# TorontoDeepLearning/convnet

Measured on NVIDIA H100. Metric: images/sec ImageNet AlexNet training, higher is better.
Workload: dtype bf16

## Files before the change

convnet_b200/csrc/conv_tc.cu:

```cuda
#include <cuda.h>
#include <cuda_bf16.h>
#include <cudaTypedefs.h>

#include <algorithm>
#include <vector>

#include "conv_kernels.h"
#include "sm90_ptx.cuh"

namespace cnb {

namespace {

constexpr int kConsumerWarps = 8;
template <int SW> constexpr int kThreadsFor = 32 * (kConsumerWarps + 1 + SW);
constexpr int BM = 128;
constexpr int BN_MAX = 128;
constexpr int BK = 32;
constexpr int kMaxStages = 8;
constexpr uint32_t kAStageBytes = BM * 128;
constexpr uint32_t kBStageBytes = BN_MAX * 128;

enum Op { kFprop = 0, kDgrad = 1, kWgrad = 2 };

struct TcParams {
  int bf16, chunk, chunk_shift, cpt, bk, nbc;
  int N, nb;
  int W, H, modX, modY, modules;
  int Cin, Cout;
  int kx, ky, sx, sy, px, py, taps;
  int frames, frame0;
  int BN, stages;
  int m_tiles, n_tiles, num_tiles;
  int kc_blocks;
  int x_mode, x_yblocks, x_ct;
  const float* xw;
  uint32_t bank_bytes;
  uint32_t epi_bytes;
  uint32_t b_tx_bytes;
  int a_merged, b_merged;
  int untied;
  int total_chunks;
  int splits, units_per_split;
  long long part_stride;
// ... 181 lines not shown
  ptx::wgmma_fence_operands(acc);
}

__device__ __forceinline__ uint32_t epi_off(int row, int col) {
  return (uint32_t)(col * (BM * 4) + ((((row >> 2) ^ col) & 7) << 4) + (((row >> 2) & ~7) << 4) + ((row & 3) << 2));
}

constexpr int kWgradPassCols = 32;
constexpr uint32_t kWgradWarpBytes = 16 * kWgradPassCols * 4;
constexpr uint32_t kWgradStageBytes = kConsumerWarps * kWgradWarpBytes;
__device__ __forceinline__ uint32_t wgrad_stage_off(int row, int col) {
  return (uint32_t)(col * 64 + ((((row >> 2) ^ (col >> 1)) & 3) << 4) + ((row & 3) << 2));
}

__device__ __forceinline__ float4 ld4(const float* a, bool vec) {
  if (vec) return *reinterpret_cast<const float4*>(a);
  return make_float4(a[0], a[1], a[2], a[3]);
}
__device__ __forceinline__ float4 ldg4(const float* a, bool vec) {
  if (vec) return __ldg(reinterpret_cast<const float4*>(a));
  return make_float4(__ldg(a), __ldg(a + 1), __ldg(a + 2), __ldg(a + 3));
}

template <int OP, bool SIG, int SW>
__device__ __forceinline__ void store_tiles(const TcParams& p, SmemCtl* ctl, uint32_t stg, int sw, int lane) {
  constexpr int kStoreWarps = SW;
  constexpr int kEpiCols = (SW == 3 && !SIG) ? 8 : 4;
  const bool vec = p.vec != 0;
  const int lr = 4 * lane;
  const int per_frame = (OP == kFprop) ? p.modules : p.W * p.H;
  const long long col_stride = (long long)p.N * (OP == kFprop ? p.out_plane : (long long)per_frame);
  const bool direct_scale = p.splits == 1;
  const float so_eff = direct_scale ? p.so : 1.f;
  const bool rmw = direct_scale && p.st != 0.f;
  uint32_t phase = 0;
  for (int t = blockIdx.x; t < p.num_tiles; t += gridDim.x) {
    const Tile tile = decode_tile<OP>(p, t);
    long long row = -1;
    const int q = tile.m_tile * p.cpt + (lr >> p.chunk_shift);
    if (q < p.total_chunks) {
      const int ib = q % p.nbc, rr = q / p.nbc, pos = rr % per_frame, f = rr / per_frame;
      const int n = ib * p.chunk + (lr & (p.chunk - 1));
      if (n < p.N) {
        if (OP == kFprop) {
          const int i = pos % p.modX, j = pos / p.modX;
          const long long pix = (long long)(i * p.o_sx + p.o_x0) + (long long)p.o_W * (j * p.o_sy + p.o_y0);
          row = f * p.out_frame_step + n + (long long)p.N * pix;
        } else {
          row = n + (long long)p.N * pos;
        }
        row += col_stride * ((long long)tile.n_tile * p.BN) + tile.split * p.part_stride;
      }
    }
    const int ncols = min(p.BN, (OP == kFprop ? p.Cout : p.Cin) - tile.n_tile * p.BN);
    const float* bias = (OP == kFprop && p.bias) ? p.bias + tile.n_tile * p.BN : nullptr;
    int bias_step = 1;
    if (OP == kFprop && p.bias && p.untied) {
      bias = p.bias + (tile.m_tile * p.cpt / p.nbc) + (long long)p.modules * tile.n_tile * p.BN;
      bias_step = p.modules;
    }
    const int mine = ncols > sw ? (ncols - sw + kStoreWarps - 1) / kStoreWarps : 0;
    const int batches = (mine + kEpiCols - 1) / kEpiCols;
    static_assert(BN_MAX <= 64 * kStoreWarps, "two bias values per lane cover a store warp's columns");
    constexpr bool kBiasHi = BN_MAX > 32 * kStoreWarps;
    float bias_lo = 0.f, bias_hi = 0.f;
    if (OP == kFprop && bias) {
      const int ca = sw + kStoreWarps * lane, cb = ca + kStoreWarps * 32;
      if (ca < ncols) bias_lo = __ldg(bias + ca * bias_step);
      if (kBiasHi && cb < ncols) bias_hi = __ldg(bias + cb * bias_step);
    }
    float4 acc[kEpiCols], old[kEpiCols], msk[kEpiCols];
    auto load_batch = [&](int b) {
      const int c0 = sw + kStoreWarps * kEpiCols * b;
#pragma unroll
      for (int k = 0; k < kEpiCols; k++) {
        const int col = c0 + kStoreWarps * k;
        old[k] = msk[k] = make_float4(0.f, 0.f, 0.f, 0.f);
        if (row < 0 || col >= ncols) continue;
        const long long idx = row + col_stride * col;
        if (rmw) old[k] = ld4(p.out + idx, vec);
        if (p.mask) msk[k] = ldg4(p.mask + idx, vec);
      }
    };
    if (batches > 0) load_batch(0);
    ptx::mbar_wait(&ctl->epi_full, phase);
    if (batches == 0 && lane == 0) ptx::mbar_arrive(&ctl->epi_empty);
    for (int b = 0; b < batches; b++) {
// ... 53 lines not shown
          *reinterpret_cast<float4*>(dst) = acc[k];
        } else {
#pragma unroll
          for (int e = 0; e < 4; e++) dst[e] = v[e];
        }
        if (p.out16) {
          __nv_bfloat16* const d16 = p.out16 + idx;
          const __nv_bfloat162 lo = __floats2bfloat162_rn(v[0], v[1]), hi = __floats2bfloat162_rn(v[2], v[3]);
          if (vec) {
            uint2 w;
            w.x = *reinterpret_cast<const uint32_t*>(&lo);
            w.y = *reinterpret_cast<const uint32_t*>(&hi);
            *reinterpret_cast<uint2*>(d16) = w;
          } else {
            d16[0] = lo.x; d16[1] = lo.y; d16[2] = hi.x; d16[3] = hi.y;
          }
        }
      }
    }
    phase ^= 1;
  }
}

template <int OP, bool BF16, bool SIG, int SW>
__global__ void __launch_bounds__(kThreadsFor<SW>, 1)
tc_conv_kernel(const __grid_constant__ CUtensorMap mapA, const __grid_constant__ CUtensorMap mapB, const __grid_constant__ TcParams p) {
  extern __shared__ uint8_t smem_raw[];
  uint8_t* smem = reinterpret_cast<uint8_t*>((reinterpret_cast<uintptr_t>(smem_raw) + 1023) & ~uintptr_t(1023));
  uint8_t* smemA = smem;
  uint8_t* smemB = smem + (size_t)p.stages * kAStageBytes;
  uint8_t* smemE = smemB + (p.bank_bytes ? (size_t)p.bank_bytes : (size_t)p.stages * kBStageBytes);
  SmemCtl* ctl = reinterpret_cast<SmemCtl*>(smemE + p.epi_bytes);

  const int warp = __shfl_sync(0xffffffffu, (int)(threadIdx.x >> 5), 0), lane = threadIdx.x & 31;

  if (threadIdx.x == 0) {
    for (int s = 0; s < p.stages; s++) { ptx::mbar_init(&ctl->full[s], 1); ptx::mbar_init(&ctl->empty[s], kConsumerWarps); }
    ptx::mbar_init(&ctl->epi_full, kConsumerWarps);
    ptx::mbar_init(&ctl->epi_empty, SW);
    ptx::fence_barrier_init();
    ptx::tma_prefetch_desc(&mapA);
    ptx::tma_prefetch_desc(&mapB);
  }
  __syncthreads();
  ptx::pdl_launch_dependents();
  ptx::pdl_wait();

  if (warp > kConsumerWarps) {
    if constexpr (OP != kWgrad) store_tiles<OP, SIG, SW>(p, ctl, ptx::smem_u32(smemE), warp - kConsumerWarps - 1, lane);
    return;
  }
  if (warp == kConsumerWarps) {
    if (lane != 0) return;
    int stage = 0; uint32_t phase = 0;
    const uint32_t tx_bytes = kAStageBytes + p.b_tx_bytes;
    for (int t = blockIdx.x; t < p.num_tiles; t += gridDim.x) {
      const Tile tile = decode_tile<OP>(p, t);
      auto begin_stage = [&]() -> uint8_t* {
        ptx::mbar_wait(&ctl->empty[stage], phase ^ 1);
        ptx::mbar_arrive_expect_tx(&ctl->full[stage], tx_bytes);
        return smemA + (size_t)stage * kAStageBytes;
      };
      auto lda5 = [&](const void* m, void* dst, int c0, int c1, int c2, int c3, int c4) {
        ptx::tma_load_5d(m, &ctl->full[stage], dst, c0, c1, c2, c3, c4);
      };
      auto lda4 = [&](const void* m, void* dst, int c0, int c1, int c2, int c3) {
        ptx::tma_load_4d(m, &ctl->full[stage], dst, c0, c1, c2, c3);
      };
      auto lda3 = [&](const void* m, void* dst, int c0, int c1, int c2) {
        ptx::tma_load_3d(m, &ctl->full[stage], dst, c0, c1, c2);
      };
      auto end_stage = [&]() { if (++stage == p.stages) { stage = 0; phase ^= 1; } };
// ... 8 lines not shown
        }
        if (p.x_mode) {
          for (int c = 0; c < p.Cin; c++)
            for (int yb = 0; yb < p.x_yblocks; yb++) {
              uint8_t* a = begin_stage();
              if (p.a_merged) {
                lda5(&mapA, a, 0, cX[0], cY[0] + 4 * yb, ch.n[0] >> 5, c);
              } else {
#pragma unroll
                for (int q = 0; q < 4; q++)
                  lda5(&mapA, a + q * (BK * 128), ch.n[q], c, cX[q], cY[q] + 4 * yb, ch.f[q]);
              }
              end_stage();
            }
        } else {
          const int cb0 = p.splits > 1 ? tile.split * p.units_per_split : 0;
          const int cb1 = p.splits > 1 ? min(cb0 + p.units_per_split, p.kc_blocks) : p.kc_blocks;
          const int mod = ch.pos[0];
          for (int ty = 0; ty < p.ky; ty++)
            for (int tx = 0; tx < p.kx; tx++) {
              const int tap = tx + p.kx * ty;
              for (int cb = cb0; cb < cb1; cb++) {
                uint8_t* a = begin_stage();
                uint8_t* b = smemB + (size_t)stage * kBStageBytes;
                if (p.a_merged) {
                  lda5(&mapA, a, 0, cb * p.bk, ch.n[0] >> p.chunk_shift, cX[0] + tx, cY[0] + ty);
                } else {
#pragma unroll
                  for (int c = 0; c < 4; c++)
                    if (c < p.cpt) lda5(&mapA, a + c * (p.bk * 128), ch.n[c], cb * p.bk, cX[c] + tx, cY[c] + ty, ch.f[c]);
                }
                const int o0 = tile.n_tile * p.BN;
                if (p.b_merged) {
                  if (p.untied) lda5(&mapB, b, 0, cb * p.bk, o0 >> p.chunk_shift, tap, mod);
                  else lda4(&mapB, b, 0, cb * p.bk, o0 >> p.chunk_shift, tap);
                } else {
                  for (int j = 0; j < ((p.BN + p.chunk - 1) >> p.chunk_shift); j++) {
                    if (p.untied) lda4(&mapB, b + j * (p.bk * 128), o0 + j * p.chunk, tap, cb * p.bk, mod);
                    else lda3(&mapB, b + j * (p.bk * 128), o0 + j * p.chunk, tap, cb * p.bk);
                  }
                }
                end_stage();
              }
            }
        }
      } else if (OP == kDgrad) {
        const Chunks ch = decode_chunks(p, tile.m_tile, p.W * p.H);
        const DgradTaps taps = dgrad_taps(p, ch);
        const bool none = dgrad_live_taps(p, taps) == 0;
        int cX[4], cY[4];
#pragma unroll
        for (int c = 0; c < 4; c++) { cX[c] = ch.pos[c] % p.W; cY[c] = ch.pos[c] / p.W; }
        const int ob0 = p.splits > 1 ? tile.split * p.units_per_split : 0;
        const int ob1 = p.splits > 1 ? min(ob0 + p.units_per_split, p.kc_blocks) : p.kc_blocks;
        for (int ty = 0; ty < p.ky; ty++)
          for (int tx = 0; tx < p.kx; tx++) {
            if (!(taps.any(tx, ty) || (none && tx == 0 && ty == 0))) continue;
            int mx[4], my[4];
#pragma unroll
            for (int c = 0; c < 4; c++) {
              const bool lv = ch.ok[c] && taps.live(c, tx, ty);
              mx[c] = lv ? (cX[c] - p.px - tx) / p.sx : -1;
              my[c] = lv ? (cY[c] - p.py - ty) / p.sy : -1;
            }
            const int tap = tx + p.kx * ty;
            const int mod = mx[0] >= 0 ? mx[0] + p.modX * my[0] : -1;
            for (int ob = ob0; ob < ob1; ob++) {
              uint8_t* a = begin_stage();
              uint8_t* b = smemB + (size_t)stage * kBStageBytes;
              if (p.a_merged) {
                lda5(&mapA, a, 0, ob * p.bk, ch.n[0] >> p.chunk_shift, mx[0], my[0]);
              } else {
#pragma unroll
                for (int c = 0; c < 4; c++)
                  if (c < p.cpt) lda5(&mapA, a + c * (p.bk * 128), ch.n[c], ob * p.bk, mx[c], my[c], p.frame0);
              }
              if (p.untied) lda4(&mapB, b, ob * p.bk, tap, tile.n_tile * p.BN, mod);
              else lda3(&mapB, b, ob * p.bk, tap, tile.n_tile * p.BN);
              end_stage();
            }
          }
      } else if (p.untied) {
        const int mx = tile.split % p.modX, my = tile.split / p.modX;
        const int X = mx * p.sx + p.px + tile.tap % p.kx, Y = my * p.sy + p.py + tile.tap / p.kx;
        for (int ib = 0; ib < p.nbc; ib++) {
          uint8_t* a = begin_stage();
          uint8_t* b = smemB + (size_t)stage * kBStageBytes;
          lda5(&mapA, a, ib * p.chunk, mx, my, tile.o_tile * BM, 0);
          lda5(&mapB, b, ib * p.chunk, X, Y, tile.c_tile * p.BN, 0);
          end_stage();
        }
      } else if (p.x_mode) {
        const int r0 = tile.split * p.units_per_split, r1 = min(r0 + p.units_per_split, p.modY * p.frames);
        const uint32_t c_bytes = (uint32_t)p.ky * 8 * 128;
        for (int r = r0; r < r1; r++) {
          const int f = r / p.modY, my = r % p.modY;
          for (int mx = 0; mx < p.modX; mx++)
            for (int ib = 0; ib < p.nb; ib++) {
              uint8_t* a = begin_stage();
              uint8_t* b = smemB + (size_t)stage * kBStageBytes;
              lda5(&mapA, a, ib * 32, mx, my, tile.o_tile * BM, f);
              for (int c = 0; c < p.x_ct; c++)
                lda5(&mapB, b + c * c_bytes, ib * 32, mx * p.sx + p.px, my * p.sy + p.py, tile.c_tile * p.x_ct + c, f);
              end_stage();
            }
        }
      } else {
        const WgradSpan sp = wgrad_span(p, tile);
        const int tx = tile.tap % p.kx, ty = tile.tap / p.kx;
        if (sp.live_rows == 0 || sp.mx_hi < sp.mx_lo) {
          for (int ib = 0; ib < p.nbc; ib++) {
            uint8_t* a = begin_stage();
            uint8_t* b = smemB + (size_t)stage * kBStageBytes;
            lda5(&mapA, a, ib * p.chunk, 0, 0, tile.o_tile * BM, 0);
            lda5(&mapB, b, ib * p.chunk, -1, -1, tile.c_tile * p.BN, 0);
            end_stage();
          }
        } else {
          for (int r = sp.r0; r < sp.r1; r++) {
            if (!wgrad_row_live(p, r, ty)) continue;
            const int f = r / p.modY, my = r % p.modY;
            const int Y = my * p.sy + p.py + ty;
            for (int mx = sp.mx_lo; mx <= sp.mx_hi; mx++) {
              const int X = mx * p.sx + p.px + tx;
              for (int ib = 0; ib < p.nbc; ib++) {
                uint8_t* a = begin_stage();
                uint8_t* b = smemB + (size_t)stage * kBStageBytes;
                lda5(&mapA, a, ib * p.chunk, mx, my, tile.o_tile * BM, f);
                lda5(&mapB, b, ib * p.chunk, X, Y, tile.c_tile * p.BN, f);
                end_stage();
              }
            }
          }
        }
      }
    }
    return;
  }

  const int g = lane >> 2, tq = lane & 3;
  const int row0 = warp * 16 + g;
  int stage = 0; uint32_t phase = 0;
  int bank_tile = -1;
  uint32_t epi_phase = 0;
  for (int t = blockIdx.x; t < p.num_tiles; t += gridDim.x) {
    const Tile tile = decode_tile<OP>(p, t);
    const int nkb = tile_kblocks<OP>(p, tile);
    float acc[BN_MAX / 8][4];
#pragma unroll
    for (int j = 0; j < BN_MAX / 8; j++)
#pragma unroll
      for (int e = 0; e < 4; e++) acc[j][e] = 0.f;

    if constexpr (BF16 || OP == kWgrad) {
      constexpr bool a_mn = (OP != kWgrad), b_mn = (OP == kFprop);
      constexpr uint32_t a_step = a_mn ? 2048u : 32u, b_step = b_mn ? 2048u : 32u;
      const uint64_t da0 = ptx::gmma_desc(ptx::smem_u32(smemA) + (uint32_t)(warp >> 2) * 8192u, a_mn ? 8192u : 16u, 1024u);
      const uint64_t db0 = ptx::gmma_desc(ptx::smem_u32(smemB), b_mn ? 8192u : 16u, 1024u);
      int prev = -1;
      ptx::wgmma_fence_operands(acc);
      for (int kb = 0; kb < nkb; kb++) {
        ptx::mbar_wait(&ctl->full[stage], phase);
        ptx::wgmma_fence();
        const uint64_t da = da0 + ((uint32_t)stage * kAStageBytes >> 4), db = db0 + ((uint32_t)stage * kBStageBytes >> 4);
#pragma unroll
        for (int ks = 0; ks < 4; ks++) {
          if constexpr (BF16)
            ptx::wgmma_m64n128k16_bf16<a_mn ? 1 : 0, b_mn ? 1 : 0>(acc, da + (ks * a_step >> 4), db + (ks * b_step >> 4));
          else
            ptx::wgmma_m64n128k8_tf32(acc, da + (ks * a_step >> 4), db + (ks * b_step >> 4));
        }
        ptx::wgmma_commit();
        ptx::wgmma_wait<1>();
        if (prev >= 0 && lane == 0) ptx::mbar_arrive(&ctl->empty[prev]);
        prev = stage;
        if (++stage == p.stages) { stage = 0; phase ^= 1; }
      }
      ptx::wgmma_wait<0>();
      ptx::wgmma_fence_operands(acc);
      if (prev >= 0 && lane == 0) ptx::mbar_arrive(&ctl->empty[prev]);
    } else if (OP == kFprop && p.x_mode) {
      if (tile.n_tile != bank_tile) {
        ptx::bar_sync(1, 32 * kConsumerWarps);
        xmode_fill_bank(p, smemB, tile.n_tile);
        ptx::fence_proxy_async_smem();
        ptx::bar_sync(1, 32 * kConsumerWarps);
        bank_tile = tile.n_tile;
      }
      const uint32_t sA = ptx::smem_u32(smemA), bank = ptx::smem_u32(smemB);
      switch (p.BN) {
        case 32: xmode_fprop_mma<32>(acc, p, ctl, sA, bank, nkb, stage, phase, row0, tq, lane); break;
        case 64: xmode_fprop_mma<64>(acc, p, ctl, sA, bank, nkb, stage, phase, row0, tq, lane); break;
        case 96: xmode_fprop_mma<96>(acc, p, ctl, sA, bank, nkb, stage, phase, row0, tq, lane); break;
        default: xmode_fprop_mma<128>(acc, p, ctl, sA, bank, nkb, stage, phase, row0, tq, lane); break;
      }
    } else {
      const uint32_t sA = ptx::smem_u32(smemA), sB = ptx::smem_u32(smemB);
      constexpr bool b_mn = (OP == kFprop);
      for (int kb = 0; kb < nkb; kb++) {
        ptx::mbar_wait(&ctl->full[stage], phase);
        const uint32_t A = sA + (uint32_t)stage * kAStageBytes, B = sB + (uint32_t)stage * kBStageBytes;
#pragma unroll
        for (int ks = 0; ks < 4; ks++) {
          const int k0 = ks * 8 + tq, k1 = k0 + 4;
          const uint32_t a0 = ptx::lds32(A + off_mnmajor(row0, k0));
          const uint32_t a1 = ptx::lds32(A + off_mnmajor(row0 + 8, k0));
          const uint32_t a2 = ptx::lds32(A + off_mnmajor(row0, k1));
          const uint32_t a3 = ptx::lds32(A + off_mnmajor(row0 + 8, k1));
#pragma unroll
          for (int j = 0; j < BN_MAX / 8; j++) {
            if (j * 8 >= p.BN) break;
            const int n = j * 8 + g;
            const uint32_t b0 = ptx::lds32(B + (b_mn ? off_mnmajor(n, k0) : off_kmajor(n, k0)));
            const uint32_t b1 = ptx::lds32(B + (b_mn ? off_mnmajor(n, k1) : off_kmajor(n, k1)));
            ptx::mma_tf32_16x8x8(acc[j], a0, a1, a2, a3, b0, b1);
          }
        }
        __syncwarp();
        if (lane == 0) ptx::mbar_arrive(&ctl->empty[stage]);
        if (++stage == p.stages) { stage = 0; phase ^= 1; }
      }
    }

    if constexpr (OP != kWgrad) {
      ptx::mbar_wait(&ctl->epi_empty, epi_phase ^ 1);
      uint32_t base[2][2];
#pragma unroll
      for (int h = 0; h < 2; h++)
#pragma unroll
        for (int e = 0; e < 2; e++) base[h][e] = ptx::smem_u32(smemE) + epi_off(row0 + 8 * h, 2 * tq + e);
#pragma unroll
      for (int j = 0; j < BN_MAX / 8; j++) {
        if (j * 8 >= p.BN) break;
#pragma unroll
        for (int h = 0; h < 2; h++)
#pragma unroll
          for (int e = 0; e < 2; e++) ptx::sts32(base[h][e] + j * 8 * BM * 4, acc[j][2 * h + e]);
      }
      __syncwarp();
      if (lane == 0) ptx::mbar_arrive(&ctl->epi_full);
      epi_phase ^= 1;
    } else if (p.epi_bytes) {
      const uint32_t stg = ptx::smem_u32(smemE) + (uint32_t)warp * kWgradWarpBytes;
      const int r4 = 4 * (lane & 3);
      const int o = tile.o_tile * BM + warp * 16 + r4;
      const long long col_stride = (long long)p.Cout * p.taps;
      float* const rp = p.out + (long long)tile.split * p.Cout * p.taps * p.Cin + o + (long long)p.Cout * tile.tap +
                        col_stride * ((long long)tile.c_tile * p.BN);
      const int ncols_valid = min(p.BN, p.Cin - tile.c_tile * p.BN);
      const bool direct_scale = (p.splits == 1) || p.untied;
      const float so_eff = direct_scale ? p.so : 1.f;
      const bool rmw = direct_scale && p.st != 0.f;
#pragma unroll
      for (int pass = 0; pass < BN_MAX / kWgradPassCols; pass++) {
        if (pass * kWgradPassCols >= p.BN) break;
// ... 97 lines not shown
  if ((reinterpret_cast<uintptr_t>(base) & 15) != 0) return false;
  for (int i = 0; i < rank; i++) {
    if (dims[i] <= 0 || dims[i] > 0xFFFFFFFFLL) return false;
    gdim[i] = (cuuint64_t)dims[i];
    bdim[i] = (cuuint32_t)box[i];
    estr[i] = 1;
    if (box[i] > 256) return false;
    if (i > 0) {
      const long long bytes = strides[i - 1] * e.esz;
      if (bytes % 16 != 0 || bytes <= 0 || bytes >= (1LL << 40)) return false;
      gstr[i - 1] = (cuuint64_t)bytes;
    }
  }
  CUresult r = encode_fn()(map, e.bf16 ? CU_TENSOR_MAP_DATA_TYPE_BFLOAT16 : CU_TENSOR_MAP_DATA_TYPE_FLOAT32, (cuuint32_t)rank,
                           const_cast<void*>(base), gdim, gstr, bdim, estr, CU_TENSOR_MAP_INTERLEAVE_NONE,
                           CU_TENSOR_MAP_SWIZZLE_128B, CU_TENSOR_MAP_L2_PROMOTION_L2_256B, CU_TENSOR_MAP_FLOAT_OOB_FILL_NONE);
  if (r != CUDA_SUCCESS) {
    fprintf(stderr, "convnet_b200: cuTensorMapEncodeTiled failed (%d)\n", (int)r);
    return false;
  }
  return true;
}

int pick_bn(int cols, int granule) {
  const int tiles = ceil_div(cols, BN_MAX);
  const int bn = ceil_div(ceil_div(cols, tiles), granule) * granule;
  return std::min(BN_MAX, std::max(granule, bn));
}

size_t smem_bytes_for(int stages, uint32_t bank_bytes, uint32_t epi_bytes) {
  const size_t b = bank_bytes ? (size_t)bank_bytes : (size_t)stages * kBStageBytes;
  return 1024 + (size_t)stages * kAStageBytes + b + epi_bytes + sizeof(SmemCtl) + 16;
}
constexpr size_t kSmemBudget = 227 * 1024;
inline uint32_t epi_bytes_for(int bn) { return (uint32_t)BM * bn * 4; }

int pick_stages(uint32_t bank_bytes, uint32_t epi_bytes) {
  int s = kMaxStages;
  while (s > 2 && smem_bytes_for(s, bank_bytes, epi_bytes) > kSmemBudget) s--;
  return s;
}

int pick_store_warps(int kblocks, double tile_bytes) {
  const double mma_us = 0.3 * kblocks;
  const double epi_us = tile_bytes / (3e6 / 132);
  return 2.0 * epi_us >= mma_us ? 7 : 3;
}

template <int OP, bool BF16, bool SIG, int SW>
void launch_one(const CUtensorMap& a, const CUtensorMap& b, const TcParams& p, size_t smem) {
  smem_opt_in(tc_conv_kernel<OP, BF16, SIG, SW>, 227 * 1024);
  const int grid = std::min(p.num_tiles, num_sms());
  launch_pdl(tc_conv_kernel<OP, BF16, SIG, SW>, dim3((unsigned)grid), dim3(kThreadsFor<SW>), smem, state().stream, a, b, p);
}

template <int OP>
void launch(const CUtensorMap& a, const CUtensorMap& b, TcParams& p) {
  auto aligned = [](const void* q, uintptr_t a) { return (reinterpret_cast<uintptr_t>(q) & (a - 1)) == 0; };
  if (OP == kWgrad) p.epi_bytes = (!p.x_mode && p.Cout % 4 == 0 && aligned(p.out, 16)) ? kWgradStageBytes : 0u;
  else p.epi_bytes = epi_bytes_for(p.BN);
  p.stages = pick_stages(p.bank_bytes, p.epi_bytes);
  const size_t smem = smem_bytes_for(p.stages, p.bank_bytes, p.epi_bytes);
  p.vec = aligned(p.out, 16) && aligned(p.mask, 16) && aligned(p.out16, 8) ? 1 : 0;
  const bool sig = p.act == kActLogistic || (p.mask && p.mask_act == kActLogistic);
  CNB_REQUIRE(OP != kWgrad || !sig, "tc_conv: wgrad has no activation epilogue");
  void (*run)(const CUtensorMap&, const CUtensorMap&, const TcParams&, size_t) = nullptr;
  if constexpr (OP != kWgrad) {
    const int kcb = p.splits > 1 ? p.units_per_split : p.kc_blocks;
    const int kblocks = (OP == kFprop && p.x_mode) ? p.Cin * p.x_yblocks : p.taps * kcb;
    const double bytes = BM * p.BN * (4.0 + (p.out16 ? 2 : 0) + (p.mask ? 4 : 0) + (p.st != 0.f && p.splits == 1 ? 4 : 0));
    if (pick_store_warps(kblocks, bytes) == 7) {
      if (sig) run = p.bf16 ? launch_one<OP, true, true, 7> : launch_one<OP, false, true, 7>;
      else run = p.bf16 ? launch_one<OP, true, false, 7> : launch_one<OP, false, false, 7>;
    } else if (sig) {
      run = p.bf16 ? launch_one<OP, true, true, 3> : launch_one<OP, false, true, 3>;
    }
  }
  if (!run) run = p.bf16 ? launch_one<OP, true, false, 3> : launch_one<OP, false, false, 3>;
  run(a, b, p, smem);
  count_launch();
  CNB_LAUNCH_CHECK("tc_conv");
}

void fill_common(TcParams& p, const ConvGeom& g, const Elem& e) {
  p.bf16 = e.bf16; p.chunk = e.chunk; p.chunk_shift = e.shift; p.cpt = BM / e.chunk; p.bk = e.bk;
  p.N = g.N; p.nb = ceil_div(g.N, 32); p.nbc = ceil_div(g.N, e.chunk);
  p.W = g.W; p.H = g.H; p.modX = g.modX; p.modY = g.modY; p.modules = g.modules;
  p.Cin = g.Cin; p.Cout = g.Cout;
  p.kx = g.kx; p.ky = g.ky; p.sx = g.sx; p.sy = g.sy; p.px = g.px; p.py = g.py; p.taps = g.kx * g.ky;
  p.frames = g.frames; p.frame0 = 0;
  p.splits = 1; p.units_per_split = 0; p.part_stride = 0;
  p.x_mode = 0; p.x_yblocks = 0; p.x_ct = 0; p.b_tx_bytes = 0;
  p.xw = nullptr; p.bank_bytes = 0; p.epi_bytes = 0;
  p.a_merged = 0; p.b_merged = 0;
// ... 97 lines not shown
             st, so, bias, per_channel / 4, act, (const float4*)mask, mask_act);
  count_launch();
  CNB_LAUNCH_CHECK("reduce_split");
}
void set_tiles(TcParams& p, int total_chunks, int cols, int k_channels) {
  p.kc_blocks = ceil_div(k_channels, p.bk);
  p.total_chunks = total_chunks;
  p.m_tiles = ceil_div(p.total_chunks, p.cpt);
  p.n_tiles = ceil_div(cols, p.BN);
  p.num_tiles = p.m_tiles * p.n_tiles;
  p.b_tx_bytes = p.x_mode ? 0u : (uint32_t)p.BN * 128;
}
size_t split_k(TcParams& p, const ConvGeom& g, long long out_elems, bool allowed) {
  if (!allowed || p.x_mode || p.taps != 1 || g.frames != 1 || out_elems % 4 != 0) return 0;
  if (p.num_tiles * 2 > num_sms() || p.kc_blocks < 8) return 0;
  const int ks = std::max(std::min(num_sms() / p.num_tiles, p.kc_blocks / 4), 1);
  if (ks > 1) {
    p.units_per_split = ceil_div(p.kc_blocks, ks);
    p.splits = ceil_div(p.kc_blocks, p.units_per_split);
    p.part_stride = out_elems;
    p.num_tiles *= p.splits;
  }
  return p.splits > 1 ? align_up(sizeof(float) * out_elems * p.splits) : 0;
}

}

static ConvOutcome tc_conv_up_impl(const ConvGeom& g, const float* images, const float* filters, float* targets, float st,
                                   float so, const Fuse& fuse, __nv_bfloat16* out16, bool bf) {
  const Elem e = elem_for(bf);
  if (g.N % 4 != 0 || g.Cout % 4 != 0) return {};
  const bool x_mode = g.Cin < 8;
  if (x_mode && (g.kx > 8 || g.ky > 8)) return {};
  if (bf && (x_mode || g.N % 8 != 0 || g.Cout % 8 != 0 || !aligned16(images) || !aligned16(filters))) return {};
  if (!g.conv && (g.N % 128 != 0 || g.frames != 1 || x_mode)) return {};
  const long long flt_n = filter_elems(g);
  if (bf && (long long)g.N * g.modules * g.frames < 1024 && !bf16_staged(filters, flt_n)) return {};
  TcParams p; fill_common(p, g, e);
  p.BN = pick_bn(g.Cout, e.chunk);
  p.x_mode = x_mode ? 1 : 0;
  p.x_yblocks = ceil_div(g.ky, 4);
  if (x_mode) {
    auto bank_bytes = [&](int bn) { return (uint32_t)g.Cin * p.x_yblocks * bn * 128; };
    while (p.BN > 32 && smem_bytes_for(3, bank_bytes(p.BN), epi_bytes_for(p.BN)) > kSmemBudget) p.BN = ceil_div(p.BN / 2, 32) * 32;
    p.bank_bytes = bank_bytes(p.BN);
    p.xw = filters;
  }
  const long long chunks = (long long)p.nb * g.modules * g.frames;
  if (chunks * 4 >= (1LL << 31)) return {};
  set_tiles(p, p.nbc * g.modules * g.frames, g.Cout, g.Cin);
  float* const out = targets + (long long)g.cout0 * g.modules * g.N;
  const float* const bias = fuse.bias ? fuse.bias + (long long)g.cout0 * (g.conv ? 1 : g.modules) : nullptr;
  const long long out_elems = (long long)g.Cout * g.modules * g.N;
  const size_t part_bytes = split_k(p, g, out_elems, g.conv);
  p.out = out;
  p.st = st; p.so = so;
  p.bias = bias; p.act = fuse.act;
  CUtensorMap ma, mb;
  const CallBuffers buf = call_buffers(bf, part_bytes, {images, g.img_total, (long long)g.cin0 * g.H * g.W * g.N},
                                       {filters, flt_n, 0});
  const long long taps = (long long)g.kx * g.ky;
  if (p.splits > 1) { p.out = buf.part; p.bias = nullptr; p.act = 0; }
  const bool emit = out16 != nullptr && p.splits == 1 && g.cout0 == 0 && g.Cout == g.CoutT;
  if (emit) p.out16 = out16;
  const bool drop = fuse.drop_scale != 0.f && p.splits == 1 && g.frames == 1 && g.cout0 == 0 && g.Cout == g.CoutT;
  if (drop) { p.drop_prob = fuse.drop_prob; p.drop_scale = fuse.drop_scale; p.drop_seed = fuse.drop_seed; }
  p.a_merged = (g.frames == 1 && g.N % 128 == 0) ? 1 : 0;
  p.b_merged = (g.Cout % e.chunk == 0) ? 1 : 0;
  if (x_mode) {
    const long long N = g.N;
    if (p.a_merged) {
      if (!merged_image_map(&ma, buf.x, e, g, g.W, g.H, g.Cin, true)) return {};
    } else {
      const long long adims[5] = {N, g.Cin, g.W, g.H, g.frames};
      const long long astr[4] = {N * g.W * g.H, N, N * g.W, g.in_frame_step};
      const int abox[5] = {32, 1, 8, 4, 1};
      if (!make_map(&ma, buf.x, e, 5, adims, astr, abox)) return {};
    }
    mb = ma;
  } else {
    if (p.a_merged) {
      if (!merged_image_map(&ma, buf.x, e, g, g.W, g.H, g.Cin, false)) return {};
    } else if (!image_map(&ma, buf.x, e, g, g.W, g.H, g.Cin, g.in_frame_step, true, e.bk)) return {};
    if (!filter_map(&mb, buf.y, e, g.Cout, taps, g.Cin, p.BN, p.b_merged, g.conv ? 0 : g.modules)) return {};
  }
  launch<kFprop>(ma, mb, p);
  if (p.splits > 1)
    reduce_split(buf.part, out, out_elems, p.splits, st, so, bias, (long long)g.modules * g.N, fuse.act, nullptr, 0);
  return {bf ? kPathTcBf16 : kPathTcTf32, emit, drop};
// ... 28 lines not shown
                                         float so, const Fuse& fuse, __nv_bfloat16* out16) {
  DgradBanks banks;
  if (!dgrad_as_fprop_eligible(g, derivs, filters, &banks)) return {};
  const Elem e = elem_for(true);
  const __nv_bfloat16* sd = bf16_staged(derivs, g.out_total);
  if (!sd) {
    __nv_bfloat16* tmp = (__nv_bfloat16*)workspace(align_up((size_t)g.out_total * 2));
    to_bf16(derivs, tmp, g.out_total);
    sd = tmp;
  }
  const __nv_bfloat16* bank = dgrad_weights(filters, g, banks, false);
  for (int i = 0; i < banks.count; i++) {
    const DgradPhase& P = banks.phase[i];
    TcParams p; fill_common(p, g, e);
    p.modX = P.Wp; p.modY = P.Hp; p.modules = P.Wp * P.Hp;
    p.W = g.modX; p.H = g.modY;
    p.kx = P.ku; p.ky = P.kv; p.taps = P.ku * P.kv; p.sx = p.sy = 1; p.px = P.px; p.py = P.py;
    p.Cin = g.Cout; p.Cout = g.Cin;
    p.BN = pick_bn(g.Cin, 64);
    set_tiles(p, p.nbc * p.modules, g.Cin, g.Cout);
    p.out = targets; p.st = 0.f; p.so = so;
    p.mask = fuse.act_state; p.mask_act = fuse.state_act; p.out16 = out16;
    p.o_sx = g.sx; p.o_sy = g.sy; p.o_x0 = P.a; p.o_y0 = P.b; p.o_W = g.W; p.out_plane = (long long)g.W * g.H;
    p.a_merged = 1;
    p.b_merged = (g.Cin % 64 == 0) ? 1 : 0;
    CUtensorMap fa, fb;
    if (!merged_image_map(&fa, sd, e, g, g.modX, g.modY, g.Cout, false) ||
        !filter_map(&fb, bank + P.offset, e, g.Cin, p.taps, g.Cout, p.BN, p.b_merged)) {
      CNB_REQUIRE(i == 0, "dgrad-as-fprop: tensor map failed after the first phase");
      return {};
    }
    launch<kFprop>(fa, fb, p);
  }
  return {kPathTcBf16, out16 != nullptr, false};
}

static ConvOutcome tc_conv_down_impl(const ConvGeom& g, const float* derivs, const float* filters, float* targets, float st,
                                     float so, const Fuse& fuse, __nv_bfloat16* out16, bool bf) {
  const Elem e = elem_for(bf);
  if (g.N % 4 != 0 || g.Cout % 4 != 0 || g.Cout < 8 || g.Cin < 8) return {};
  if (bf && (g.N % 8 != 0 || g.Cout % 8 != 0 || !aligned16(derivs) || !aligned16(filters))) return {};
  if (!g.conv && (g.N % 128 != 0 || g.frames != 1)) return {};
  const long long flt_n = filter_elems(g);
  if (bf && (long long)g.N * g.W * g.H < 1024 && !bf16_staged(filters, flt_n)) return {};
  TcParams p; fill_common(p, g, e);
  p.BN = pick_bn(g.Cin, 16);
// ... 130 lines not shown
```

convnet_b200/csrc/sm90_ptx.cuh:

```cuda
#pragma once
#include <cuda_runtime.h>
#include <stdint.h>

namespace cnb {
namespace ptx {

__device__ __forceinline__ uint32_t smem_u32(const void* p) {
  return static_cast<uint32_t>(__cvta_generic_to_shared(p));
}

__device__ __forceinline__ void mbar_init(uint64_t* bar, uint32_t count) {
  asm volatile("mbarrier.init.shared::cta.b64 [%0], %1;" ::"r"(smem_u32(bar)), "r"(count));
}
__device__ __forceinline__ void fence_barrier_init() {
  asm volatile("fence.mbarrier_init.release.cluster;" ::: "memory");
}
__device__ __forceinline__ void mbar_arrive_expect_tx(uint64_t* bar, uint32_t bytes) {
  asm volatile("mbarrier.arrive.expect_tx.shared::cta.b64 _, [%0], %1;" ::"r"(smem_u32(bar)), "r"(bytes) : "memory");
}
__device__ __forceinline__ void mbar_arrive(uint64_t* bar) {
  asm volatile("mbarrier.arrive.shared::cta.b64 _, [%0];" ::"r"(smem_u32(bar)) : "memory");
}
__device__ __forceinline__ bool mbar_try_wait(uint64_t* bar, uint32_t parity) {
  uint32_t ok;
// ... 64 lines not shown
  asm volatile("ld.shared.v4.f32 {%0, %1, %2, %3}, [%4];" : "=f"(v.x), "=f"(v.y), "=f"(v.z), "=f"(v.w) : "r"(addr) : "memory");
  return v;
}
__device__ __forceinline__ void sts32(uint32_t addr, float v) {
  asm volatile("st.shared.f32 [%0], %1;" ::"r"(addr), "f"(v) : "memory");
}

__device__ __forceinline__ void mma_tf32_16x8x8(float (&d)[4], uint32_t a0, uint32_t a1, uint32_t a2, uint32_t a3,
                                                uint32_t b0, uint32_t b1) {
  asm volatile("mma.sync.aligned.m16n8k8.row.col.f32.tf32.tf32.f32 {%0, %1, %2, %3}, {%4, %5, %6, %7}, {%8, %9}, "
               "{%0, %1, %2, %3};"
               : "+f"(d[0]), "+f"(d[1]), "+f"(d[2]), "+f"(d[3])
               : "r"(a0), "r"(a1), "r"(a2), "r"(a3), "r"(b0), "r"(b1));
}

__device__ __forceinline__ uint64_t gmma_desc(uint32_t smem_addr, uint32_t lbo_bytes, uint32_t sbo_bytes) {
  return (uint64_t)((smem_addr >> 4) & 0x3FFF) | ((uint64_t)((lbo_bytes >> 4) & 0x3FFF) << 16) |
         ((uint64_t)((sbo_bytes >> 4) & 0x3FFF) << 32) | (1ULL << 62);
}
__device__ __forceinline__ void wgmma_fence() { asm volatile("wgmma.fence.sync.aligned;" ::: "memory"); }
__device__ __forceinline__ void wgmma_commit() { asm volatile("wgmma.commit_group.sync.aligned;" ::: "memory"); }
template <int N>
__device__ __forceinline__ void wgmma_wait() { asm volatile("wgmma.wait_group.sync.aligned %0;" ::"n"(N) : "memory"); }
__device__ __forceinline__ void wgmma_fence_operands(float (&d)[16][4]) {
#pragma unroll
  for (int j = 0; j < 16; j++)
#pragma unroll
    for (int e = 0; e < 4; e++) asm volatile("" : "+f"(d[j][e])::"memory");
}

#define CNB_ACC4(j) "+f"(d[j][0]), "+f"(d[j][1]), "+f"(d[j][2]), "+f"(d[j][3])
template <int TA, int TB>
__device__ __forceinline__ void wgmma_m64n128k16_bf16(float (&d)[16][4], uint64_t desc_a, uint64_t desc_b) {
  asm volatile(
      "{\n\t.reg .pred p;\n\tsetp.ne.b32 p, %68, 0;\n\t"
      "wgmma.mma_async.sync.aligned.m64n128k16.f32.bf16.bf16 "
      "{%0, %1, %2, %3, %4, %5, %6, %7, %8, %9, %10, %11, %12, %13, %14, %15, "
      "%16, %17, %18, %19, %20, %21, %22, %23, %24, %25, %26, %27, %28, %29, %30, %31, "
      "%32, %33, %34, %35, %36, %37, %38, %39, %40, %41, %42, %43, %44, %45, %46, %47, "
      "%48, %49, %50, %51, %52, %53, %54, %55, %56, %57, %58, %59, %60, %61, %62, %63}, "
      "%64, %65, p, 1, 1, %66, %67;\n\t}"
      : CNB_ACC4(0), CNB_ACC4(1), CNB_ACC4(2), CNB_ACC4(3), CNB_ACC4(4), CNB_ACC4(5), CNB_ACC4(6), CNB_ACC4(7),
        CNB_ACC4(8), CNB_ACC4(9), CNB_ACC4(10), CNB_ACC4(11), CNB_ACC4(12), CNB_ACC4(13), CNB_ACC4(14), CNB_ACC4(15)
      : "l"(desc_a), "l"(desc_b), "n"(TA), "n"(TB), "r"(1));
}

__device__ __forceinline__ void wgmma_m64n128k8_tf32(float (&d)[16][4], uint64_t desc_a, uint64_t desc_b) {
  asm volatile(
      "{\n\t.reg .pred p;\n\tsetp.ne.b32 p, %66, 0;\n\t"
      "wgmma.mma_async.sync.aligned.m64n128k8.f32.tf32.tf32 "
      "{%0, %1, %2, %3, %4, %5, %6, %7, %8, %9, %10, %11, %12, %13, %14, %15, "
      "%16, %17, %18, %19, %20, %21, %22, %23, %24, %25, %26, %27, %28, %29, %30, %31, "
      "%32, %33, %34, %35, %36, %37, %38, %39, %40, %41, %42, %43, %44, %45, %46, %47, "
      "%48, %49, %50, %51, %52, %53, %54, %55, %56, %57, %58, %59, %60, %61, %62, %63}, "
      "%64, %65, p, 1, 1;\n\t}"
      : CNB_ACC4(0), CNB_ACC4(1), CNB_ACC4(2), CNB_ACC4(3), CNB_ACC4(4), CNB_ACC4(5), CNB_ACC4(6), CNB_ACC4(7),
        CNB_ACC4(8), CNB_ACC4(9), CNB_ACC4(10), CNB_ACC4(11), CNB_ACC4(12), CNB_ACC4(13), CNB_ACC4(14), CNB_ACC4(15)
      : "l"(desc_a), "l"(desc_b), "r"(1));
}

template <int N>
__device__ __forceinline__ void wgmma_m64nNk8_tf32_rs(float (&d)[16][4], const uint32_t (&a)[4], uint64_t desc_b) {
  static_assert(N == 32 || N == 64 || N == 96 || N == 128, "tf32 RS wgmma: N in {32, 64, 96, 128}");
  if constexpr (N == 32) {
    asm volatile(
        "{\n\t.reg .pred p;\n\tsetp.ne.b32 p, %21, 0;\n\t"
        "wgmma.mma_async.sync.aligned.m64n32k8.f32.tf32.tf32 "
        "{%0, %1, %2, %3, %4, %5, %6, %7, %8, %9, %10, %11, %12, %13, %14, %15}, "
        "{%16, %17, %18, %19}, %20, p, 1, 1;\n\t}"
// ... 46 lines not shown
```

Baseline: 17040.

## Add 192-wide N tiles for bf16 fprop/dgrad with wave-cost tile selection

Adds a wide N-tile variant (BN=192) of the warp-specialized conv kernel, using the m64n192k16 bf16 wgmma. A host-side heuristic picks 128 or 192 from a wave-count cost model. Wider tiles raise A-operand reuse and can cut tile count and waves for layers whose channel counts fit 192 (e.g. 192 or 384 channels). The cost is more accumulator registers per thread (96 floats), larger per-stage smem and so possibly fewer pipeline stages, and a bigger epilogue staging buffer.

```diff
diff --git a/convnet_b200/csrc/conv_tc.cu b/convnet_b200/csrc/conv_tc.cu
--- a/convnet_b200/csrc/conv_tc.cu
+++ b/convnet_b200/csrc/conv_tc.cu
@@ -20,6 +20,7 @@
 constexpr int kMaxStages = 8;
 constexpr uint32_t kAStageBytes = BM * 128;
 constexpr uint32_t kBStageBytes = BN_MAX * 128;
+constexpr int kWideBN = 192;
 
 enum Op { kFprop = 0, kDgrad = 1, kWgrad = 2 };
 
@@ -247,7 +248,7 @@
   return make_float4(__ldg(a), __ldg(a + 1), __ldg(a + 2), __ldg(a + 3));
 }
 
-template <int OP, bool SIG, int SW>
+template <int OP, bool SIG, int SW, int NB>
 __device__ __forceinline__ void store_tiles(const TcParams& p, SmemCtl* ctl, uint32_t stg, int sw, int lane) {
   constexpr int kStoreWarps = SW;
   constexpr int kEpiCols = (SW == 3 && !SIG) ? 8 : 4;
@@ -286,8 +287,8 @@
     }
     const int mine = ncols > sw ? (ncols - sw + kStoreWarps - 1) / kStoreWarps : 0;
     const int batches = (mine + kEpiCols - 1) / kEpiCols;
-    static_assert(BN_MAX <= 64 * kStoreWarps, "two bias values per lane cover a store warp's columns");
-    constexpr bool kBiasHi = BN_MAX > 32 * kStoreWarps;
+    static_assert(NB <= 64 * kStoreWarps, "two bias values per lane cover a store warp's columns");
+    constexpr bool kBiasHi = NB > 32 * kStoreWarps;
     float bias_lo = 0.f, bias_hi = 0.f;
     if (OP == kFprop && bias) {
       const int ca = sw + kStoreWarps * lane, cb = ca + kStoreWarps * 32;
@@ -387,14 +388,16 @@
   }
 }
 
-template <int OP, bool BF16, bool SIG, int SW>
+template <int OP, bool BF16, bool SIG, int SW, int NB = BN_MAX>
 __global__ void __launch_bounds__(kThreadsFor<SW>, 1)
 tc_conv_kernel(const __grid_constant__ CUtensorMap mapA, const __grid_constant__ CUtensorMap mapB, const __grid_constant__ TcParams p) {
+  static_assert(NB == BN_MAX || (NB == kWideBN && OP == kFprop && BF16 && !SIG && SW == 3), "wide tiles: the bf16 fprop SW = 3 instance");
+  constexpr uint32_t kBStage = NB * 128;
   extern __shared__ uint8_t smem_raw[];
   uint8_t* smem = reinterpret_cast<uint8_t*>((reinterpret_cast<uintptr_t>(smem_raw) + 1023) & ~uintptr_t(1023));
   uint8_t* smemA = smem;
   uint8_t* smemB = smem + (size_t)p.stages * kAStageBytes;
-  uint8_t* smemE = smemB + (p.bank_bytes ? (size_t)p.bank_bytes : (size_t)p.stages * kBStageBytes);
+  uint8_t* smemE = smemB + (p.bank_bytes ? (size_t)p.bank_bytes : (size_t)p.stages * kBStage);
   SmemCtl* ctl = reinterpret_cast<SmemCtl*>(smemE + p.epi_bytes);
 
   const int warp = __shfl_sync(0xffffffffu, (int)(threadIdx.x >> 5), 0), lane = threadIdx.x & 31;
@@ -412,7 +415,7 @@
   ptx::pdl_wait();
 
   if (warp > kConsumerWarps) {
-    if constexpr (OP != kWgrad) store_tiles<OP, SIG, SW>(p, ctl, ptx::smem_u32(smemE), warp - kConsumerWarps - 1, lane);
+    if constexpr (OP != kWgrad) store_tiles<OP, SIG, SW, NB>(p, ctl, ptx::smem_u32(smemE), warp - kConsumerWarps - 1, lane);
     return;
   }
   if (warp == kConsumerWarps) {
@@ -467,7 +470,7 @@
               const int tap = tx + p.kx * ty;
               for (int cb = cb0; cb < cb1; cb++) {
                 uint8_t* a = begin_stage();
-                uint8_t* b = smemB + (size_t)stage * kBStageBytes;
+                uint8_t* b = smemB + (size_t)stage * kBStage;
                 if (p.a_merged) {
                   lda5(&mapA, a, 0, cb * p.bk, ch.n[0] >> p.chunk_shift, cX[0] + tx, cY[0] + ty);
                 } else {
@@ -512,7 +515,7 @@
             const int mod = mx[0] >= 0 ? mx[0] + p.modX * my[0] : -1;
             for (int ob = ob0; ob < ob1; ob++) {
               uint8_t* a = begin_stage();
-              uint8_t* b = smemB + (size_t)stage * kBStageBytes;
+              uint8_t* b = smemB + (size_t)stage * kBStage;
               if (p.a_merged) {
                 lda5(&mapA, a, 0, ob * p.bk, ch.n[0] >> p.chunk_shift, mx[0], my[0]);
               } else {
@@ -530,7 +533,7 @@
         const int X = mx * p.sx + p.px + tile.tap % p.kx, Y = my * p.sy + p.py + tile.tap / p.kx;
         for (int ib = 0; ib < p.nbc; ib++) {
           uint8_t* a = begin_stage();
-          uint8_t* b = smemB + (size_t)stage * kBStageBytes;
+          uint8_t* b = smemB + (size_t)stage * kBStage;
           lda5(&mapA, a, ib * p.chunk, mx, my, tile.o_tile * BM, 0);
           lda5(&mapB, b, ib * p.chunk, X, Y, tile.c_tile * p.BN, 0);
           end_stage();
@@ -543,7 +546,7 @@
           for (int mx = 0; mx < p.modX; mx++)
             for (int ib = 0; ib < p.nb; ib++) {
               uint8_t* a = begin_stage();
-              uint8_t* b = smemB + (size_t)stage * kBStageBytes;
+              uint8_t* b = smemB + (size_t)stage * kBStage;
               lda5(&mapA, a, ib * 32, mx, my, tile.o_tile * BM, f);
               for (int c = 0; c < p.x_ct; c++)
                 lda5(&mapB, b + c * c_bytes, ib * 32, mx * p.sx + p.px, my * p.sy + p.py, tile.c_tile * p.x_ct + c, f);
@@ -556,7 +559,7 @@
         if (sp.live_rows == 0 || sp.mx_hi < sp.mx_lo) {
           for (int ib = 0; ib < p.nbc; ib++) {
             uint8_t* a = begin_stage();
-            uint8_t* b = smemB + (size_t)stage * kBStageBytes;
+            uint8_t* b = smemB + (size_t)stage * kBStage;
             lda5(&mapA, a, ib * p.chunk, 0, 0, tile.o_tile * BM, 0);
             lda5(&mapB, b, ib * p.chunk, -1, -1, tile.c_tile * p.BN, 0);
             end_stage();
@@ -570,7 +573,7 @@
               const int X = mx * p.sx + p.px + tx;
               for (int ib = 0; ib < p.nbc; ib++) {
                 uint8_t* a = begin_stage();
-                uint8_t* b = smemB + (size_t)stage * kBStageBytes;
+                uint8_t* b = smemB + (size_t)stage * kBStage;
                 lda5(&mapA, a, ib * p.chunk, mx, my, tile.o_tile * BM, f);
                 lda5(&mapB, b, ib * p.chunk, X, Y, tile.c_tile * p.BN, f);
                 end_stage();
@@ -591,9 +594,9 @@
   for (int t = blockIdx.x; t < p.num_tiles; t += gridDim.x) {
     const Tile tile = decode_tile<OP>(p, t);
     const int nkb = tile_kblocks<OP>(p, tile);
-    float acc[BN_MAX / 8][4];
-#pragma unroll
-    for (int j = 0; j < BN_MAX / 8; j++)
+    float acc[NB / 8][4];
+#pragma unroll
+    for (int j = 0; j < NB / 8; j++)
 #pragma unroll
       for (int e = 0; e < 4; e++) acc[j][e] = 0.f;
 
@@ -607,11 +610,11 @@
       for (int kb = 0; kb < nkb; kb++) {
         ptx::mbar_wait(&ctl->full[stage], phase);
         ptx::wgmma_fence();
-        const uint64_t da = da0 + ((uint32_t)stage * kAStageBytes >> 4), db = db0 + ((uint32_t)stage * kBStageBytes >> 4);
+        const uint64_t da = da0 + ((uint32_t)stage * kAStageBytes >> 4), db = db0 + ((uint32_t)stage * kBStage >> 4);
 #pragma unroll
         for (int ks = 0; ks < 4; ks++) {
           if constexpr (BF16)
-            ptx::wgmma_m64n128k16_bf16<a_mn ? 1 : 0, b_mn ? 1 : 0>(acc, da + (ks * a_step >> 4), db + (ks * b_step >> 4));
+            ptx::wgmma_m64nNk16_bf16<NB, a_mn ? 1 : 0, b_mn ? 1 : 0>(acc, da + (ks * a_step >> 4), db + (ks * b_step >> 4));
           else
             ptx::wgmma_m64n128k8_tf32(acc, da + (ks * a_step >> 4), db + (ks * b_step >> 4));
         }
@@ -644,7 +647,7 @@
       constexpr bool b_mn = (OP == kFprop);
       for (int kb = 0; kb < nkb; kb++) {
         ptx::mbar_wait(&ctl->full[stage], phase);
-        const uint32_t A = sA + (uint32_t)stage * kAStageBytes, B = sB + (uint32_t)stage * kBStageBytes;
+        const uint32_t A = sA + (uint32_t)stage * kAStageBytes, B = sB + (uint32_t)stage * kBStage;
 #pragma unroll
         for (int ks = 0; ks < 4; ks++) {
           const int k0 = ks * 8 + tq, k1 = k0 + 4;
@@ -675,7 +678,7 @@
 #pragma unroll
         for (int e = 0; e < 2; e++) base[h][e] = ptx::smem_u32(smemE) + epi_off(row0 + 8 * h, 2 * tq + e);
 #pragma unroll
-      for (int j = 0; j < BN_MAX / 8; j++) {
+      for (int j = 0; j < NB / 8; j++) {
         if (j * 8 >= p.BN) break;
 #pragma unroll
         for (int h = 0; h < 2; h++)
@@ -819,36 +822,46 @@
   return true;
 }
 
-int pick_bn(int cols, int granule) {
-  const int tiles = ceil_div(cols, BN_MAX);
+int pick_bn(int cols, int granule, int bn_max = BN_MAX) {
+  const int tiles = ceil_div(cols, bn_max);
   const int bn = ceil_div(ceil_div(cols, tiles), granule) * granule;
-  return std::min(BN_MAX, std::max(granule, bn));
-}
-
-size_t smem_bytes_for(int stages, uint32_t bank_bytes, uint32_t epi_bytes) {
-  const size_t b = bank_bytes ? (size_t)bank_bytes : (size_t)stages * kBStageBytes;
+  return std::min(bn_max, std::max(granule, bn));
+}
+
+inline uint32_t b_stage_bytes(int bn) { return bn > BN_MAX ? (uint32_t)bn * 128 : kBStageBytes; }
+size_t smem_bytes_for(int stages, uint32_t bank_bytes, uint32_t epi_bytes, uint32_t b_stage = kBStageBytes) {
+  const size_t b = bank_bytes ? (size_t)bank_bytes : (size_t)stages * b_stage;
   return 1024 + (size_t)stages * kAStageBytes + b + epi_bytes + sizeof(SmemCtl) + 16;
 }
 constexpr size_t kSmemBudget = 227 * 1024;
 inline uint32_t epi_bytes_for(int bn) { return (uint32_t)BM * bn * 4; }
 
-int pick_stages(uint32_t bank_bytes, uint32_t epi_bytes) {
+int pick_stages(uint32_t bank_bytes, uint32_t epi_bytes, uint32_t b_stage = kBStageBytes) {
   int s = kMaxStages;
-  while (s > 2 && smem_bytes_for(s, bank_bytes, epi_bytes) > kSmemBudget) s--;
+  while (s > 2 && smem_bytes_for(s, bank_bytes, epi_bytes, b_stage) > kSmemBudget) s--;
   return s;
 }
 
-int pick_store_warps(int kblocks, double tile_bytes) {
-  const double mma_us = 0.3 * kblocks;
+int pick_store_warps(int kblocks, double tile_bytes, int bn) {
+  const double mma_us = 0.3 * kblocks * std::max(bn, BN_MAX) / BN_MAX;
   const double epi_us = tile_bytes / (3e6 / 132);
   return 2.0 * epi_us >= mma_us ? 7 : 3;
 }
 
-template <int OP, bool BF16, bool SIG, int SW>
+template <int OP>
+int plan_store_warps(const TcParams& p) {
+  const int kcb = p.splits > 1 ? p.units_per_split : p.kc_blocks;
+  const int kblocks = (OP == kFprop && p.x_mode) ? p.Cin * p.x_yblocks : p.taps * kcb;
+  const double bytes = BM * p.BN * (4.0 + (p.out16 ? 2 : 0) + (p.mask ? 4 : 0) + (p.st != 0.f && p.splits == 1 ? 4 : 0));
+  return pick_store_warps(kblocks, bytes, p.BN);
+}
+inline bool plan_sig(const TcParams& p) { return p.act == kActLogistic || (p.mask && p.mask_act == kActLogistic); }
+
+template <int OP, bool BF16, bool SIG, int SW, int NB = BN_MAX>
 void launch_one(const CUtensorMap& a, const CUtensorMap& b, const TcParams& p, size_t smem) {
-  smem_opt_in(tc_conv_kernel<OP, BF16, SIG, SW>, 227 * 1024);
+  smem_opt_in(tc_conv_kernel<OP, BF16, SIG, SW, NB>, 227 * 1024);
   const int grid = std::min(p.num_tiles, num_sms());
-  launch_pdl(tc_conv_kernel<OP, BF16, SIG, SW>, dim3((unsigned)grid), dim3(kThreadsFor<SW>), smem, state().stream, a, b, p);
+  launch_pdl(tc_conv_kernel<OP, BF16, SIG, SW, NB>, dim3((unsigned)grid), dim3(kThreadsFor<SW>), smem, state().stream, a, b, p);
 }
 
 template <int OP>
@@ -856,17 +869,18 @@
   auto aligned = [](const void* q, uintptr_t a) { return (reinterpret_cast<uintptr_t>(q) & (a - 1)) == 0; };
   if (OP == kWgrad) p.epi_bytes = (!p.x_mode && p.Cout % 4 == 0 && aligned(p.out, 16)) ? kWgradStageBytes : 0u;
   else p.epi_bytes = epi_bytes_for(p.BN);
-  p.stages = pick_stages(p.bank_bytes, p.epi_bytes);
-  const size_t smem = smem_bytes_for(p.stages, p.bank_bytes, p.epi_bytes);
+  p.stages = pick_stages(p.bank_bytes, p.epi_bytes, b_stage_bytes(p.BN));
+  const size_t smem = smem_bytes_for(p.stages, p.bank_bytes, p.epi_bytes, b_stage_bytes(p.BN));
   p.vec = aligned(p.out, 16) && aligned(p.mask, 16) && aligned(p.out16, 8) ? 1 : 0;
-  const bool sig = p.act == kActLogistic || (p.mask && p.mask_act == kActLogistic);
+  const bool sig = plan_sig(p);
   CNB_REQUIRE(OP != kWgrad || !sig, "tc_conv: wgrad has no activation epilogue");
   void (*run)(const CUtensorMap&, const CUtensorMap&, const TcParams&, size_t) = nullptr;
   if constexpr (OP != kWgrad) {
-    const int kcb = p.splits > 1 ? p.units_per_split : p.kc_blocks;
-    const int kblocks = (OP == kFprop && p.x_mode) ? p.Cin * p.x_yblocks : p.taps * kcb;
-    const double bytes = BM * p.BN * (4.0 + (p.out16 ? 2 : 0) + (p.mask ? 4 : 0) + (p.st != 0.f && p.splits == 1 ? 4 : 0));
-    if (pick_store_warps(kblocks, bytes) == 7) {
+    const int sw = plan_store_warps<OP>(p);
+    if (p.BN > BN_MAX) {
+      CNB_REQUIRE(OP == kFprop && p.bf16 && !sig && sw == 3 && p.BN == kWideBN, "tc_conv: wide tile outside its plan");
+      if constexpr (OP == kFprop) run = launch_one<OP, true, false, 3, kWideBN>;
+    } else if (sw == 7) {
       if (sig) run = p.bf16 ? launch_one<OP, true, true, 7> : launch_one<OP, false, true, 7>;
       else run = p.bf16 ? launch_one<OP, true, false, 7> : launch_one<OP, false, false, 7>;
     } else if (sig) {
@@ -1010,6 +1024,22 @@
     p.num_tiles *= p.splits;
   }
   return p.splits > 1 ? align_up(sizeof(float) * out_elems * p.splits) : 0;
+}
+
+void widen_n_tile(TcParams& p, int cols, int granule, int k_channels) {
+  if (!p.bf16 || p.x_mode || p.untied || p.splits > 1 || plan_sig(p) || plan_store_warps<kFprop>(p) != 3) return;
+  long long best = -1;
+  int best_bn = p.BN;
+  for (const int w : {BN_MAX, kWideBN}) {
+    const int bn = pick_bn(cols, granule, w);
+    const long long waves = ceil_div<long long>((long long)p.m_tiles * ceil_div(cols, bn), num_sms());
+    const long long cost = waves * (128 + bn);
+    if (best < 0 || cost < best) { best = cost; best_bn = bn; }
+  }
+  if (best_bn > BN_MAX) {
+    p.BN = best_bn;
+    set_tiles(p, p.total_chunks, cols, k_channels);
+  }
 }
 
 }
@@ -1053,6 +1083,7 @@
   if (emit) p.out16 = out16;
   const bool drop = fuse.drop_scale != 0.f && p.splits == 1 && g.frames == 1 && g.cout0 == 0 && g.Cout == g.CoutT;
   if (drop) { p.drop_prob = fuse.drop_prob; p.drop_scale = fuse.drop_scale; p.drop_seed = fuse.drop_seed; }
+  widen_n_tile(p, g.Cout, e.chunk, g.Cin);
   p.a_merged = (g.frames == 1 && g.N % 128 == 0) ? 1 : 0;
   p.b_merged = (g.Cout % e.chunk == 0) ? 1 : 0;
   if (x_mode) {
@@ -1127,6 +1158,7 @@
     p.out = targets; p.st = 0.f; p.so = so;
     p.mask = fuse.act_state; p.mask_act = fuse.state_act; p.out16 = out16;
     p.o_sx = g.sx; p.o_sy = g.sy; p.o_x0 = P.a; p.o_y0 = P.b; p.o_W = g.W; p.out_plane = (long long)g.W * g.H;
+    widen_n_tile(p, g.Cin, 64, g.Cout);
     p.a_merged = 1;
     p.b_merged = (g.Cin % 64 == 0) ? 1 : 0;
     CUtensorMap fa, fb;
diff --git a/convnet_b200/csrc/sm90_ptx.cuh b/convnet_b200/csrc/sm90_ptx.cuh
--- a/convnet_b200/csrc/sm90_ptx.cuh
+++ b/convnet_b200/csrc/sm90_ptx.cuh
@@ -110,9 +110,10 @@
 __device__ __forceinline__ void wgmma_commit() { asm volatile("wgmma.commit_group.sync.aligned;" ::: "memory"); }
 template <int N>
 __device__ __forceinline__ void wgmma_wait() { asm volatile("wgmma.wait_group.sync.aligned %0;" ::"n"(N) : "memory"); }
-__device__ __forceinline__ void wgmma_fence_operands(float (&d)[16][4]) {
+template <int J>
+__device__ __forceinline__ void wgmma_fence_operands(float (&d)[J][4]) {
 #pragma unroll
-  for (int j = 0; j < 16; j++)
+  for (int j = 0; j < J; j++)
 #pragma unroll
     for (int e = 0; e < 4; e++) asm volatile("" : "+f"(d[j][e])::"memory");
 }
@@ -133,6 +134,30 @@
       : "l"(desc_a), "l"(desc_b), "n"(TA), "n"(TB), "r"(1));
 }
 
+template <int TA, int TB>
+__device__ __forceinline__ void wgmma_m64n192k16_bf16(float (&d)[24][4], uint64_t desc_a, uint64_t desc_b) {
+  asm volatile(
+      "{\n\t.reg .pred p;\n\tsetp.ne.b32 p, %100, 0;\n\t"
+      "wgmma.mma_async.sync.aligned.m64n192k16.f32.bf16.bf16 "
+      "{%0, %1, %2, %3, %4, %5, %6, %7, %8, %9, %10, %11, %12, %13, %14, %15, "
+      "%16, %17, %18, %19, %20, %21, %22, %23, %24, %25, %26, %27, %28, %29, %30, %31, "
+      "%32, %33, %34, %35, %36, %37, %38, %39, %40, %41, %42, %43, %44, %45, %46, %47, "
+      "%48, %49, %50, %51, %52, %53, %54, %55, %56, %57, %58, %59, %60, %61, %62, %63, "
+      "%64, %65, %66, %67, %68, %69, %70, %71, %72, %73, %74, %75, %76, %77, %78, %79, "
+      "%80, %81, %82, %83, %84, %85, %86, %87, %88, %89, %90, %91, %92, %93, %94, %95}, "
+      "%96, %97, p, 1, 1, %98, %99;\n\t}"
+      : CNB_ACC4(0), CNB_ACC4(1), CNB_ACC4(2), CNB_ACC4(3), CNB_ACC4(4), CNB_ACC4(5), CNB_ACC4(6), CNB_ACC4(7),
+        CNB_ACC4(8), CNB_ACC4(9), CNB_ACC4(10), CNB_ACC4(11), CNB_ACC4(12), CNB_ACC4(13), CNB_ACC4(14), CNB_ACC4(15),
+        CNB_ACC4(16), CNB_ACC4(17), CNB_ACC4(18), CNB_ACC4(19), CNB_ACC4(20), CNB_ACC4(21), CNB_ACC4(22), CNB_ACC4(23)
+      : "l"(desc_a), "l"(desc_b), "n"(TA), "n"(TB), "r"(1));
+}
+template <int N, int TA, int TB>
+__device__ __forceinline__ void wgmma_m64nNk16_bf16(float (&d)[N / 8][4], uint64_t desc_a, uint64_t desc_b) {
+  static_assert(N == 128 || N == 192, "bf16 wgmma: N in {128, 192}");
+  if constexpr (N == 128) wgmma_m64n128k16_bf16<TA, TB>(d, desc_a, desc_b);
+  else wgmma_m64n192k16_bf16<TA, TB>(d, desc_a, desc_b);
+}
+
 __device__ __forceinline__ void wgmma_m64n128k8_tf32(float (&d)[16][4], uint64_t desc_a, uint64_t desc_b) {
   asm volatile(
       "{\n\t.reg .pred p;\n\tsetp.ne.b32 p, %66, 0;\n\t"
```

Measured after the change: 17440 (median of 6 runs). 1.02x the previous value.
